# tomer196/GaUDI

Measured on AMD Instinct MI355X. Metric: guided molecules/sec (1000-step), higher is better.
Workload: dtype f32

## Files before the change

### gaudi_amd/csrc/w8_edm.h

```cpp
#pragma once
#include "edm_device.h"
#include "w8_common.h"
#include "w8_split.h"
#include "w8_nodes_f16.h"

namespace gaudi {
namespace w8 {

__host__ __device__ constexpr int gn_lds_buffers(int gn) { return gn == 2 ? 2 : 0; }
template <int HP, int SP = 0, int GN = 0>
struct NetSmem {
  static constexpr bool kGlobalNodes = GN != 0;
  float *h, *p, *q;
  float *agg, *agg1;
  float* ring;
  float *x, *x0;
  uint32_t *pmax, *qmax;
  float* hsc;
  f4* geo;
  float* d0;
  float* trans;
  float* vec;
  float* hk = nullptr;
  __host__ __device__ static int floats(int N, int S) {
// ... 126 lines not shown
  __syncthreads();
  compute_geo(sm, mg, 0.f, tid, true);
  typename EdgeRing<HP, SP>::type ring;
  er_init<HP>(ring, sm.ring, W.ktail != 0, W.ws, W.hinv);
  static_assert(SP == 0 || NodeMath<SP>::kF16, "the split edge GEMMs take their column scales from the fp16 node GEMMs' row maxima");
  constexpr bool NH = NodeMath<SP>::kF16;
  constexpr bool RI = node_ring_idle(HP, SP, GN);
  constexpr bool STG = GN && !NH;
  float* const xs0 = sm.ring;
  float* const xs1 = sm.ring + stage_stride(N * LD);
  if constexpr (!RI) er_start<HP>(ring, wbe, lay.gcl(0, 0) + 2 * PK, wave, lane);
  typename NodePFSel<HP, NH>::type pf;
  node_prefetch_x<HP, NH, kAheadOne>(pf, wb, wbe, lay.gcl(0, 0), mg.NC, wave, lane, tw);
  auto hctx = [&]() {
    if constexpr (NH) {
      if constexpr (RI) return node_ctx_h<HP>(sm.ring, EdgeRing<HP, SP>::kFloats, mg.NC, W.hinv, tw, sm.hsc);
      else return node_ctx_h<HP>(ring.slot(ring.par ^ 1), EdgeRing<HP, SP>::kFloats / 2, mg.NC, W.hinv, tw, sm.hsc);
    } else {
      return NodeCtxH{1.f, nullptr, nullptr, tw, nullptr};
    }
  };
  const bool keep = NH && sm.hk != nullptr;
  bool h_kept = false;
  constexpr int NV = (7 * HP + 16 + kThreads - 1) / kThreads;
  VecPF<NV> vpf;
  vec_prefetch<NV, kThreads>(vpf, wb, lay.gcl(0, 0) + 6 * PK, 7 * HP + 16, tid);
  STAMP(ST_EDM_IO);

  for (int l = 0; l < W.L; ++l) {
    compute_geo(sm, mg, W.norm_constant, tid, false);
    STAMP(ST_GEO);
    for (int s = 0; s < W.S; ++s) {
      const int G = lay.gcl(l, s);
      const int Wnext_edge = s + 1 < W.S ? lay.gcl(l, s + 1) + 2 * PK : lay.equ(l) + 2 * PK;
      if constexpr (STG) stage_rows(xs0, sm.h, N * LD, wave, lane);
      for (int idx = tid; idx < N * (LD / 4); idx += kThreads) {
        *(f4*)(sm.agg + 4 * idx) = splat(0.f);
        *(f4*)(sm.agg1 + 4 * idx) = splat(0.f);
      }
      if (tid < N) {
        sm.pmax[tid] = 0u;
        sm.qmax[tid] = 0u;
      }
      vec_commit<NV, kThreads>(vpf, sm.vec, 7 * HP + 16, tid);
      if constexpr (STG) stage_wait();
      else __syncthreads();
      STAMP(ST_STAGE);
      const float *cr = sm.vec, *cd = sm.vec + HP, *b1 = sm.vec + 2 * HP, *b2 = sm.vec + 3 * HP, *wa = sm.vec + 4 * HP,
                  *bn1 = sm.vec + 5 * HP, *bn2 = sm.vec + 6 * HP;
      const float ba = sm.vec[7 * HP];
      const float crmax = sm.vec[7 * HP + 1], cdmax = sm.vec[7 * HP + 2];
      {
        const NodeCtxH cx = keep ? node_ctx_keep<HP>(hctx(), sm.hk, mg.NC) : hctx();
        node_gemm_x<HP, EPI_NONE, false, GN, NH, kAheadOne, kAheadAll, FL>(wb, wbe, G, sm.h, xs0, !h_kept, -1, nullptr, nullptr, b1, sm.p, nullptr, nullptr, mg.NC,
                                                      wave, lane, tw, cx, pf, G + PK, nullptr, sm.pmax);
        h_kept = keep;
        node_gemm_x<HP, EPI_NONE, false, GN, NH, kAheadAll, kAheadOne, FL>(wb, wbe, G + PK, sm.h, xs0, false, -1, nullptr, nullptr, nullptr, sm.q, nullptr,
                                                      nullptr, mg.NC, wave, lane, tw, cx, pf,
                                                      G + 3 * PK, nullptr, sm.qmax);
      }
      STAMP(ST_NODE);
      __syncthreads();
      STAMP(ST_BARRIER);
      if constexpr (RI) er_start<HP>(ring, wbe, G + 2 * PK, wave, lane);
      for (int rd = 0; rd < mg.rounds; ++rd) {
        const TileCols tc = load_tile(mg, rd, wave, c);
        const f4 gg = sm.geo[tc.slot];
        f4 acc[T];
        const float d0v = sm.d0[tc.slot];
        const float ub = __builtin_bit_cast(float, sm.pmax[tc.i]) + __builtin_bit_cast(float, sm.qmax[tc.j]) + crmax * gg[0] + cdmax * fabsf(d0v);
        er_gemm_pq<HP>(acc, ring, wbe, G + 2 * PK, rd + 1 < mg.rounds ? G + 2 * PK : (RI ? -1 : Wnext_edge), b2, cr, cd,
                         sm.p + tc.i * LD + 4 * g, sm.q + tc.j * LD + 4 * g, gg[0], d0v, ub, tc.active, wave, lane STAMP_ARGS);
        STAMP(ST_EDGE);
        if (tc.active) {
          float sdot = 0.f;
#pragma unroll
          for (int t = 0; t < T; ++t) {
            const f4 m = silu4v(acc[t]);
            acc[t] = m;
            const f4 wv = *(const f4*)(wa + 16 * t + 4 * g);
            sdot += m[0] * wv[0] + m[1] * wv[1] + m[2] * wv[2] + m[3] * wv[3];
          }
          float a = 1.f;
          if (W.attention) a = sigmoid_f(reduce_groups(sdot) + ba);
          const float sc = a * tc.mk;
#pragma unroll
          for (int t = 0; t < T; ++t) acc[t] = acc[t] * sc;
          scatter_runs<HP>(acc, tc, sm.agg, sm.agg1, g);
        }
        STAMP(ST_EDGE_EPI);
      }
      __syncthreads();
      STAMP(ST_BARRIER);
      constexpr bool SUM = NH && GN == 0;
      if constexpr (!SUM) {
        if constexpr (STG) stage_rows(xs0, sm.h, N * LD, wave, lane);
        for (int idx = tid; idx < N * (HP / 4); idx += kThreads) {
          const int n = idx / (HP / 4), f = 4 * (idx % (HP / 4));
          if constexpr (STG)
            *(f4*)(xs1 + n * LD + f) = (*(const f4*)(sm.agg + n * LD + f) + *(const f4*)(sm.agg1 + n * LD + f)) / W.normf;
          else
            *(f4*)(sm.agg + n * LD + f) = (*(const f4*)(sm.agg + n * LD + f) + *(const f4*)(sm.agg1 + n * LD + f)) / W.normf;
        }
        if constexpr (STG) stage_wait();
        else __syncthreads();
      }
      STAMP(ST_MISC);
      node_gemm_x<HP, EPI_SILU, true, GN, NH, kAheadOne, kAheadOne, FL, SUM ? 2 : 0>(
          wb, wbe, G + 3 * PK, sm.h, xs0, !h_kept, G + 4 * PK, sm.agg, xs1, bn1, sm.p, nullptr, nullptr, mg.NC, wave, lane, tw,
          keep ? node_ctx_keep<HP>(hctx(), sm.hk, mg.NC) : hctx(), pf, G + 5 * PK, nullptr, nullptr, sm.agg1, W.normf);
      STAMP(ST_NODE);
      __syncthreads();
      STAMP(ST_BARRIER);
      vec_prefetch<NV, kThreads>(vpf, wb, s + 1 < W.S ? lay.gcl(l, s + 1) + 6 * PK : lay.equ(l) + 3 * PK,
                                 s + 1 < W.S ? 7 * HP + 16 : 5 * HP + 16, tid);
      if constexpr (STG) {
        stage_rows(xs0, sm.p, N * LD, wave, lane);
        stage_wait();
      }
      node_gemm_x<HP, EPI_RESIDUAL_MASK, false, GN, NH, kAheadOne, kAheadOne, FL>(wb, wbe, G + 5 * PK, sm.p, xs0, true, -1, nullptr, nullptr, bn2, sm.h, sm.h, mg.mask,
                                                       mg.NC, wave, lane, tw, hctx(), pf,
                                                       s + 1 < W.S ? lay.gcl(l, s + 1) : lay.equ(l));
      h_kept = false;
      STAMP(ST_NODE);
      __syncthreads();
      STAMP(ST_BARRIER);
    }
    {
      const int E = lay.equ(l);
      const int Wnext_edge = l + 1 < W.L ? lay.gcl(l + 1, 0) + 2 * PK : -1;
      vec_commit<NV, kThreads>(vpf, sm.vec, 5 * HP + 16, tid);
      if (tid < N) {
        sm.pmax[tid] = 0u;
        sm.qmax[tid] = 0u;
      }
      if constexpr (STG) {
        stage_rows(xs0, sm.h, N * LD, wave, lane);
        stage_wait();
      } else {
        __syncthreads();
      }
      STAMP(ST_STAGE);
      const float *cr = sm.vec, *cd = sm.vec + HP, *b1 = sm.vec + 2 * HP, *b2 = sm.vec + 3 * HP, *w3 = sm.vec + 4 * HP;
      const float crmax = sm.vec[5 * HP], cdmax = sm.vec[5 * HP + 1];
      {
        const NodeCtxH cx = keep ? node_ctx_keep<HP>(hctx(), sm.hk, mg.NC) : hctx();
        node_gemm_x<HP, EPI_NONE, false, GN, NH, kAheadOne, kAheadAll, FL>(wb, wbe, E, sm.h, xs0, !h_kept, -1, nullptr, nullptr, b1, sm.p, nullptr, nullptr, mg.NC,
                                                      wave, lane, tw, cx, pf, E + PK, nullptr, sm.pmax);
        h_kept = keep;
// ... 96 lines not shown
```

### gaudi_amd/csrc/w8_nodes_f16.h

```cpp
#pragma once
#include "w8_split.h"

namespace gaudi {
namespace w8 {


constexpr float kLoScale = 2048.f;
#ifndef GAUDI_NODE_ABLATE
#define GAUDI_NODE_ABLATE 0
#endif
constexpr int kAblateH = GAUDI_NODE_ABLATE;
#ifndef GAUDI_NODE_STAMPS
#define GAUDI_NODE_STAMPS 0
#endif
#ifndef GAUDI_NODE_PRIO
#define GAUDI_NODE_PRIO 1
#endif
struct NodeStampH {
  unsigned long long sum[8], last;
  __device__ __forceinline__ void start() { last = __builtin_amdgcn_s_memtime(); }
  __device__ __forceinline__ void mark(int i) {
    const unsigned long long t = __builtin_amdgcn_s_memtime();
    sum[i] += t - last;
    last = t;
// ... 55 lines not shown
};
template <bool DIV>
struct RowsSum {
  const float *a, *b;
  float d;
  __device__ __forceinline__ f4 load(int off) const {
    const f4 s = *(const f4*)(a + off) + *(const f4*)(b + off);
    return DIV ? s / d : s;
  }
};
__device__ __forceinline__ RowsOne rows_of(const float* x) { return RowsOne{x}; }
__device__ __forceinline__ RowsOne rows_of(const RowsOne& r) { return r; }
__device__ __forceinline__ RowsOne rows_of(decltype(nullptr)) { return RowsOne{nullptr}; }
template <bool DIV>
__device__ __forceinline__ RowsSum<DIV> rows_of(const RowsSum<DIV>& r) { return r; }
template <int HP, class SRC>
__device__ __forceinline__ SplitRowH split_row_load(const SRC& X, int n, int lane) {
  constexpr int LD = HP + 4;
  SplitRowH r;
  r.x = lane < HP / 4 ? X.load(n * LD + 4 * lane) : splat(0.f);
  r.mx = umax(umax(absbits(r.x[0]), absbits(r.x[1])), umax(absbits(r.x[2]), absbits(r.x[3])));
  return r;
}
template <int HP>
__device__ __forceinline__ void split_row_store(const SplitBufH& sb, const f4 x, uint32_t mx, int n, int lane) {
  constexpr int T = HP / 16, nc = nh_chunks(HP);
  const int m = lane >> 3, g = (lane >> 1) & 3, half = lane & 1;
  int k = 141 - (int)(mx >> 23);
  k = k > 126 ? 126 : k;
  const float s = __builtin_bit_cast(float, (uint32_t)(k + 127) << 23), inv = __builtin_bit_cast(float, (uint32_t)(127 - k) << 23);
  const float y0 = x[0] * s, y1 = x[1] * s, y2 = x[2] * s, y3 = x[3] * s;
  const uint32_t h01 = pk_f16(y0, y1), h23 = pk_f16(y2, y3);
  const f2 f01 = unpk_f16(h01), f23 = unpk_f16(h23);
  const uint32_t l01 = pk_f16((y0 - f01[0]) * kLoScale, (y1 - f01[1]) * kLoScale),
                 l23 = pk_f16((y2 - f23[0]) * kLoScale, (y3 - f23[1]) * kLoScale);
  const int ct = n >> 4, c = n & 15;
  if (m < nc) {
    float* d = sb.chunk(m) + ct * 512 + nh_bpos(c, g) + half * 2;
    *(u2*)d = (u2){h01, h23};
    *(u2*)(d + 256) = (u2){l01, l23};
  } else if (nh_odd(HP) && lane < HP / 4) {
    float* d = sb.tail(HP) + ct * 256 + 4 * (lane - 4 * (T - 1)) * 16 + c;
    d[0] = x[0];
    d[16] = x[1];
    d[32] = x[2];
    d[48] = x[3];
  }
  if (lane == 0) sb.scale(HP)[ct * 16 + c] = inv;
}
template <int HP, class SRC>
__device__ __forceinline__ void split_rows_h(const SplitBufH& sb, const SRC& X_, int N, int wave, int lane) {
  const auto X = rows_of(X_);
  for (int n = wave; n < N; n += 2 * kWaves) {
    const int n2 = n + kWaves < N ? n + kWaves : n;
    SplitRowH a = split_row_load<HP>(X, n, lane), b = split_row_load<HP>(X, n2, lane);
    a.mx = wave_max_u32(a.mx);
    b.mx = wave_max_u32(b.mx);
    split_row_store<HP>(sb, a.x, a.mx, n, lane);
    if (n2 != n) split_row_store<HP>(sb, b.x, b.mx, n2, lane);
  }
}

__device__ __forceinline__ void lds_barrier() {
  asm volatile("s_waitcnt lgkmcnt(0)" ::: "memory");
  __builtin_amdgcn_s_barrier();
  asm volatile("" ::: "memory");
}

#ifndef GAUDI_NODE_DEPTH
#define GAUDI_NODE_DEPTH 3
#endif
#ifndef GAUDI_NODE_LATE
#define GAUDI_NODE_LATE 0
#endif
#ifndef GAUDI_NODE_TAIL_EARLY
#define GAUDI_NODE_TAIL_EARLY 0
#endif
template <int HP>
struct NodeGeoH {
  static constexpr int T = HP / 16;
  static constexpr int NTW = T > kWaves ? 2 : 1;
  static constexpr int nc = nh_chunks(HP);
  static constexpr int D = nc < GAUDI_NODE_DEPTH ? (nc > 0 ? nc : 1) : GAUDI_NODE_DEPTH;
  static constexpr bool odd = nh_odd(HP);
};
template <int NTW>
struct NodeSetH {
  u4 p[NTW][2];
};
template <int HP>
struct NodePFH {
// ... 22 lines not shown
template <int HP, int AHEAD = kAheadAll>
__device__ __forceinline__ void node_prefetch_h(NodePFH<HP>& pf, const WBuf& wh, int W , int wave, int lane) {
  constexpr int nd = AHEAD < NodeGeoH<HP>::D ? AHEAD : NodeGeoH<HP>::D;
  const TileLanesH<HP> tl(wave, lane);
  static_for<nd>([&](auto d_tag) {
    constexpr int d = decltype(d_tag)::value;
    nh_load<HP>(pf.s[d], wh, 2 * W + d * nh_chunk_floats(HP), tl);
  });
}

constexpr int kNodePlain = 0;
constexpr int kNodeFresh = 1;
constexpr int kNodeOneTile = 2;
constexpr int kTailRuntime = 0;
constexpr int kTailOne = 1;

struct NodeCtxH {
  float winv;
  float* split_a;
  float* split_b;
  bool ktail;
  float* scales;
  float* scales_b = nullptr;
};

struct YInitBias {};
struct YInitRows {
  const float* y;
};
template <int HP, int EPI, bool TWO, int MAXNT, int PIN = kAheadOne, int POUT = kAheadOne, int FL = kNodePlain, int TAIL = kTailRuntime,
          int NU = 0, class XB = const float*, class XA = const float*, class YI = YInitBias>
__device__ __forceinline__ void node_gemm_h(const WBuf& wh, int Wa, const XA& sXa, bool do_split_a, int Wb, const XB& sXb,
                                            const float* sBias, float* sY, const float* sRes, const float* sMask, int N, int wave,
                                            int lane, const NodeCtxH& cx, NodePFH<HP>& pf, int nextW = -1, float* gPre = nullptr,
                                            uint32_t* sMaxOut = nullptr ,
                                            NodeStampH* ns = nullptr, const YI& yinit = YI{}) {
  (void)ns;
  (void)yinit;
  using G = NodeGeoH<HP>;
  constexpr int T = G::T, LD = HP + 4, NTW = NU > 0 ? NU : G::NTW, nc = G::nc, D = G::D;
  constexpr int kIn = PIN < D ? PIN : D, kOut = POUT < D ? POUT : D;
  constexpr int kLate = nc < D ? 0 : (GAUDI_NODE_LATE < kOut ? GAUDI_NODE_LATE : kOut);
  constexpr int TQ = TAIL == kTailOne ? 1 : 4;
  const bool ktail = TAIL == kTailOne ? true : cx.ktail;
  constexpr bool kFresh = FL == kNodeFresh;
  const int c = lane & 15, g = lane >> 4;
  const int nt = (MAXNT < 2 || N <= 16) ? 1 : (MAXNT < 3 || N <= 32) ? 2 : 3;
  const bool seq = TWO && cx.split_b == cx.split_a;
  const SplitBufH sa{cx.split_a, nt, cx.scales}, sb{cx.split_b, nt, cx.scales_b != nullptr ? cx.scales_b : cx.scales + kScaleFloatsH};
  const int bpos = nh_bpos(c, g);
  const TileLanesH<HP> tl(wave, lane);
  const TileLanesH<HP> tl_next(wave, lane, nextW >= 0);
  const int Wn = nextW >= 0 ? nextW : Wa;
  static_for<D>([&](auto d_tag) {
    constexpr int d = decltype(d_tag)::value;
    if constexpr (d >= kIn) nh_load<HP, NTW>(pf.s[d], wh, 2 * Wa + d * nh_chunk_floats(HP), tl);
  });
  float ta[NTW][TQ], tb[NTW][TQ];
  if constexpr (G::odd) {
#pragma unroll
    for (int u = 0; u < NTW; ++u) {
      const int t = wave + kWaves * u < T ? wave + kWaves * u : 0;
#pragma unroll
      for (int q = 0; q < TQ; ++q) {
        const int ln = ((q == 0 || !ktail) && wave + kWaves * u < T) ? lane : kOOBLane;
        ta[u][q] = __builtin_bit_cast(float, __builtin_amdgcn_raw_buffer_load_b32(wh.r, ln * 4, (2 * Wa + nh_tail_off(HP) + t * 256 + q * 64) * 4, 0));
        if constexpr (TWO)
          tb[u][q] = __builtin_bit_cast(float, __builtin_amdgcn_raw_buffer_load_b32(wh.r, ln * 4, (2 * Wb + nh_tail_off(HP) + t * 256 + q * 64) * 4, 0));
      }
    }
  }
  NSTAMP(0);
  if (!(kAblateH & 1)) {
    const int ls = kFresh ? fresh(lane) : lane;
    if (do_split_a) split_rows_h<HP>(sa, rows_of(sXa), N, wave, ls);
    if (TWO && !seq) split_rows_h<HP>(sb, sXb, N, wave, ls);
    NSTAMP(1);
    if (do_split_a || (TWO && !seq)) lds_barrier();
    NSTAMP(2);
  }

  f4 acc0[MAXNT][NTW], acc1[MAXNT][NTW], y[MAXNT][NTW];
#pragma unroll
  for (int j = 0; j < MAXNT; ++j)
#pragma unroll
    for (int u = 0; u < NTW; ++u) {
      const int t = wave + kWaves * u < T ? wave + kWaves * u : 0;
      acc0[j][u] = splat(0.f);
      acc1[j][u] = splat(0.f);
      y[j][u] = sBias != nullptr ? *(const f4*)(sBias + 16 * t + 4 * g) : splat(0.f);
      if constexpr (std::is_same<YI, YInitRows>::value)
        y[j][u] = j * 16 + c < N ? *(const f4*)(yinit.y + (j * 16 + c) * LD + 16 * t + 4 * g) : splat(0.f);
    }
  struct BH {
    u4 h, l;
  };
  auto bld = [&](const SplitBufH& s_, int i, int j) {
    const float* q = s_.chunk(i) + bpos + j * 512;
    return BH{*(const u4*)q, *(const u4*)(q + 256)};
  };
  auto mm = [&](const NodeSetH<G::NTW>& s, const BH& b, int j) {
// ... 93 lines not shown
  source(std::integral_constant<int, 0>{}, sa);
  NSTAMP(4);
  if constexpr (!TWO) late(std::integral_constant<int, kOut - kLate>{});
  fold(sa, ta);
  NSTAMP(5);
  if constexpr (TWO) {
    if (seq) {
      lds_barrier();
      split_rows_h<HP>(sb, sXb, N, wave, kFresh ? fresh(lane) : lane);
      lds_barrier();
    }
    tail_early(sb, tb);
    source(std::integral_constant<int, 1>{}, sb);
    late(std::integral_constant<int, kOut - kLate>{});
    fold(sb, tb);
  }
  static_for<D>([&](auto d_tag) {
    if constexpr (decltype(d_tag)::value > kOut - kLate) late(d_tag);
  });
#if GAUDI_NODE_PRIO
  if constexpr (!kFresh) __builtin_amdgcn_s_setprio(0);
#endif
  const int le = kFresh ? fresh(lane) : lane, ce = le & 15, ge = le >> 4;
  static_for<MAXNT>([&](auto j_tag) {
    constexpr int j = decltype(j_tag)::value;
    if (j < nt) {
#pragma unroll
      for (int u = 0; u < NTW; ++u) {
        const int t = wave + kWaves * u;
        const int nd = j * 16 + ce;
        f4 yy = y[j][u];
        if (t < T && nd < N) {
          float* dst = sY + nd * LD + 16 * t + 4 * ge;
          const bool pad = G::odd && ktail && t == T - 1 && ge > 0;
          if (pad) yy = splat(0.f);
          if (gPre != nullptr) nstash_store((f4*)(gPre + nd * HP + 16 * t + 4 * ge), yy);
          if (sMaxOut != nullptr) atomicMax(sMaxOut + nd, umax(umax(absbits(yy[0]), absbits(yy[1])), umax(absbits(yy[2]), absbits(yy[3]))));
          if (!pad) {
            if (EPI == EPI_SILU) yy = silu4v(yy);
            if (EPI == EPI_RESIDUAL_MASK) {
              const f4 r = *(const f4*)(sRes + nd * LD + 16 * t + 4 * ge);
              yy = (r + yy) * sMask[nd];
            }
            if (EPI == EPI_MUL_DSILU) {
              const f4 r = *(const f4*)(sRes + nd * LD + 16 * t + 4 * ge);
              yy = yy * dsilu4v(r);
            }
            if (EPI == EPI_ACCUM) yy = *(const f4*)(sRes + nd * LD + 16 * t + 4 * ge) + yy;
          }
          *(f4*)dst = yy;
        }
      }
    }
  });
  NSTAMP(6);
}

template <int HP>
struct SideGeoH {
  static constexpr int T = HP / 16, nc = nh_chunks(HP), TG = 7;
  static constexpr int NG = (T + TG - 1) / TG;
  static constexpr int kSteps = NG * nc;
  static constexpr bool odd = nh_odd(HP);
  static_assert(nc >= 1, "at least one fp16 chunk");
  __host__ __device__ static constexpr int tiles(int gq) { return (gq + 1) * TG <= T ? TG : T - gq * TG; }
  __host__ __device__ static constexpr int loads(int s) {
    return (s < 0 || s >= kSteps) ? 0 : tiles(s / nc) * (2 + ((odd && s % nc == nc - 1) ? 1 : 0));
  }
};
template <int HP>
struct SideJobH {
  using G = SideGeoH<HP>;
  u4 w[G::TG][2];
// ... 82 lines not shown
  });
}

#ifndef GAUDI_NODE_F16
#define GAUDI_NODE_F16 1
#endif
template <int SP>
struct NodeMath {
  static constexpr bool kF16 = SP != 0 && GAUDI_NODE_F16 != 0;
};
template <int HP, bool NH>
struct NodePFSel {
  using type = NodePF<HP>;
};
template <int HP>
struct NodePFSel<HP, true> {
  using type = NodePFH<HP>;
};
template <int HP, bool NH, int AHEAD, class PF>
__device__ __forceinline__ void node_prefetch_x(PF& pf, const WBuf& wb, const WBuf& wbe, int W, int N, int wave, int lane, bool tw) {
  if constexpr (NH) node_prefetch_h<HP, AHEAD>(pf, wbe, W, wave, lane);
  else node_prefetch<HP>(pf, wb, W, wave, lane, tw);
}
template <int HP, int EPI, bool TWO, int GN, bool NH, int PIN, int POUT, int FL = kNodePlain, int XBS = 0, class PF>
__device__ __forceinline__ void node_gemm_x(const WBuf& wb, const WBuf& wbe, int Wa, const float* Xa, const float* XaS, bool split_a, int Wb,
                                            const float* Xb, const float* XbS, const float* sBias, float* sY, const float* sRes,
                                            const float* sMask, int N, int wave, int lane, bool tw, const NodeCtxH& cx, PF& pf,
                                            int nextW = -1, float* gPre = nullptr, uint32_t* sMaxOut = nullptr,
                                            const float* Xb1 = nullptr, float xb_div = 1.f) {
  static_assert(XBS == 0 || (NH && GN == 0 && TWO), "summed second sources: the fp16-pair form of the resident kernels");
  if constexpr (NH) {
    constexpr int MAXNT = GN ? 3 : FL == kNodeOneTile ? 1 : 2;
    constexpr int TAIL = FL == kNodeOneTile && nh_odd(HP) ? kTailOne : kTailRuntime;
    if constexpr (XBS == 0)
      node_gemm_h<HP, EPI, TWO, MAXNT, PIN, POUT, FL, TAIL>(wbe, Wa, Xa, split_a, Wb, Xb, sBias, sY, sRes, sMask, N, wave, lane, cx, pf, nextW,
                                                            gPre, sMaxOut);
    else
      node_gemm_h<HP, EPI, TWO, MAXNT, PIN, POUT, FL, TAIL>(wbe, Wa, Xa, split_a, Wb, RowsSum<XBS == 2>{Xb, Xb1, xb_div}, sBias, sY, sRes, sMask, N,
                                                            wave, lane, cx, pf, nextW, gPre, sMaxOut);
  } else if constexpr (GN != 0) {
    node_gemm_n<HP, EPI, true, 3>(wb, Wa, XaS, Wb, XbS, sBias, sY, sRes, sMask, N, wave, lane, tw, &pf, nextW, gPre);
  } else {
    node_gemm<HP, EPI, true>(wb, Wa, Xa, Wb, Xb, sBias, sY, sRes, sMask, N, wave, lane, tw, &pf, nextW, gPre);
  }
}
__host__ __device__ constexpr bool node_ring_idle(int HP, int SP, bool GN) {
  return GN || (SP != 0 && GAUDI_NODE_F16 != 0 && (SP == 2 || HP < 48));
}
template <int HP>
__device__ __forceinline__ NodeCtxH node_ctx_h(float* region, int cap, int N, float winv, bool ktail, float* scales) {
  const int nct = N <= 16 ? 1 : N <= 32 ? 2 : 3;
  const int need = nh_split_floats(HP, nct);
  return NodeCtxH{winv, region, 2 * need <= cap ? region + need : region, ktail, scales};
}
__host__ __device__ constexpr int nh_keep_floats(int HP, int N) { return nh_split_floats(HP, N <= 16 ? 1 : N <= 32 ? 2 : 3) + kScaleFloatsH; }
template <int HP>
__device__ __forceinline__ NodeCtxH node_ctx_keep(const NodeCtxH& cx, float* keep, int N) {
  const int nct = N <= 16 ? 1 : N <= 32 ? 2 : 3;
  return NodeCtxH{cx.winv, keep + kScaleFloatsH, cx.split_a, cx.ktail, keep, cx.scales};
  (void)nct;
}

// ... 3 lines not shown
```

### gaudi_amd/csrc/w8_pred.h

```cpp
#pragma once
#include "pred_device.h"
#include "w8_edm.h"

namespace gaudi {
namespace w8 {

template <int HP, int SP = 0, int GN = 0, bool PG = false>
struct PredSmem {
  static_assert(!(PG && GN != 0), "PG is a variant of the resident kernels");
  static_assert(!GN || SP != 0, "global node buffers: split edge GEMMs only (the fp32 form's publish buffer starts in b0 / b1)");
  static constexpr bool kGlobalNodes = GN != 0;
  float *b2, *b3, *b4;
  float *b0, *b1;
  float* ring;
  float* pub;
  float *x, *x0, *dx;
  uint32_t *pmax, *qmax;
  float* hsc;
  f4* geo;
  float *d0, *trans, *dd0;
  float* pred;
  float* vec;
  float* hk = nullptr;
  float* side = nullptr;
// ... 76 lines not shown
    }
  }
  __syncthreads();
  compute_geo(sm, mg, 0.f, tid, true);
  typename EdgeRing<HP, SP>::type ring;
  er_init<HP>(ring, sm.ring, W.ktail != 0, W.ws, W.hinv);
  constexpr bool NH = NodeMath<SP>::kF16;
  constexpr bool RI = node_ring_idle(HP, SP, GN);
  constexpr bool STG = GN && !NH;
  float* const xs0 = sm.ring;
  float* const xs1 = sm.ring + stage_stride(N * LD);
  if constexpr (!RI) er_start<HP>(ring, wbe, lay.layer(0) + 2 * HP * HP, wave, lane);
  typename NodePFSel<HP, NH>::type pf;
  node_prefetch_x<HP, NH, kAheadOne>(pf, wb, wbe, lay.layer(0), mg.NC, wave, lane, tw);
  auto hctx = [&]() {
    if constexpr (NH) {
      if constexpr (RI) return node_ctx_h<HP>(sm.ring, EdgeRing<HP, SP>::kFloats, mg.NC, W.hinv, tw, sm.hsc);
      else return node_ctx_h<HP>(ring.slot(ring.par ^ 1), EdgeRing<HP, SP>::kFloats / 2, mg.NC, W.hinv, tw, sm.hsc);
    } else {
      return NodeCtxH{1.f, nullptr, nullptr, tw, nullptr};
    }
  };
  const bool keep = NH && sm.hk != nullptr;
  constexpr bool kSideA = (SD & 1) != 0;
  static_assert(!kSideA || (NH && !MR && GN == 0 && !RI && FL == kNodeOneTile), "the side job is a form of the resident N1 kernel");
  constexpr int NV = (PredLayerW::vec_count(HP) + kThreads - 1) / kThreads;
  VecPF<NV> vpf;
  vec_prefetch<NV, kThreads>(vpf, wb, PredLayerW::vec_off(lay.layer(0), HP), PredLayerW::vec_count(HP), tid);

  for (int l = 0; l < W.L; ++l) {
    const bool last = l == W.L - 1;
    const PredLayerW Lw(w, lay.layer(l), HP, sm.vec);
    const bool side_l = kSideA && sm.side != nullptr && !last && (tw || !SplitGeo<HP, SP == 0 ? 1 : SP>::kTailOK);
    vec_commit<NV, kThreads>(vpf, sm.vec, PredLayerW::vec_count(HP), tid);
    if constexpr (STG) stage_rows(xs0, h, N * LD, wave, lane);
    for (int idx = tid; idx < N * LD; idx += kThreads) {
      agg[idx] = 0.f;
      agg1[idx] = 0.f;
    }
    if (tid < N) {
      sm.pmax[tid] = 0u;
      sm.qmax[tid] = 0u;
    }
    float* st = stash + (size_t)l * (3 * N * HP + 4 * N);
    for (int idx = tid; idx < N; idx += kThreads) gstore4((f4*)(st + 3 * N * HP) + idx, *(const f4*)(sm.x + 4 * idx));
    compute_geo(sm, mg, 1.0f, tid, false);
    if constexpr (STG) stage_wait();
    else __syncthreads();
    STAMP(ST_STAGE);
    {
      const NodeCtxH cx = keep ? node_ctx_keep<HP>(hctx(), sm.hk, mg.NC) : hctx();
      node_gemm_x<HP, EPI_NONE, false, GN, NH, kAheadOne, kAheadAll, FL>(wb, wbe, Lw.A, h, xs0, true, -1, nullptr, nullptr, Lw.b1, p, nullptr, nullptr, mg.NC, wave,
                                                    lane, tw, cx, pf, Lw.Bm, nullptr, sm.pmax);
      node_gemm_x<HP, EPI_NONE, false, GN, NH, kAheadAll, kAheadOne, FL>(wb, wbe, Lw.Bm, h, xs0, false, -1, nullptr, nullptr, nullptr, q, nullptr, nullptr, mg.NC,
                                                    wave, lane, tw, cx, pf, side_l ? Lw.Wn1a : Lw.Wn1h, nullptr, sm.qmax);
    }
    STAMP(ST_NODE);
    __syncthreads();
    STAMP(ST_BARRIER);
    if constexpr (RI) er_start<HP>(ring, wbe, Lw.W2, wave, lane);
    for (int idx = tid; idx < N * (HP / 4); idx += kThreads) {
      const int n = idx / (HP / 4), f = 4 * (idx % (HP / 4));
      nstash_store((f4*)st + idx, *(const f4*)(p + n * LD + f));
      nstash_store((f4*)(st + N * HP) + idx, *(const f4*)(q + n * LD + f));
    }
    STAMP(ST_STASH);
    int rd = 0;
    if (side_l && wave == kWaves - 1) {
      if constexpr (kSideA) {
        constexpr int n = side_trip_count<HP, SP>();
        SideJobH<HP> job;
        const SideArgsH sa{wbe, Lw.Wn1h, Lw.bn1, SplitBufH{sm.hk + kScaleFloatsH, 1, sm.hk}, W.hinv, sm.side, mg.NC};
        side_issue<HP, 0>(job, sa, lane);
        side_trips<HP, SP, 0>(ring, wbe, split_off(Lw.W2), split_off(Lw.Wc1), lane, job, sa);
        side_trips<HP, SP, n>(ring, wbe, split_off(Lw.Wc1), split_off(lay.layer(l + 1) + 2 * HP * HP), lane, job, sa);
        side_rest<HP, 2 * n>(job, sa, lane);
      }
    } else
    {
    pred_fwd_round:
      const bool more = MR && rd + 1 < mg.rounds;
      const TileCols tc = load_tile(mg, MR ? rd : 0, wave, c);
      const f4 gg = sm.geo[tc.slot];
// ... 53 lines not shown
        if (++rd < mg.rounds) goto pred_fwd_round;
      }
    }
    __syncthreads();
    STAMP(ST_BARRIER);
    constexpr bool SUM = NH && GN == 0;
    if constexpr (!SUM) {
      if constexpr (STG) stage_rows(xs0, h, N * LD, wave, lane);
      for (int idx = tid; idx < N * (HP / 4); idx += kThreads) {
        const int n = idx / (HP / 4), f = 4 * (idx % (HP / 4));
        if constexpr (STG)
          *(f4*)(xs1 + n * LD + f) = *(const f4*)(agg + n * LD + f) + *(const f4*)(agg1 + n * LD + f);
        else
          *(f4*)(agg + n * LD + f) = *(const f4*)(agg + n * LD + f) + *(const f4*)(agg1 + n * LD + f);
      }
      if constexpr (STG) stage_wait();
      else __syncthreads();
    }
    STAMP(ST_MISC);
    if constexpr (kSideA) {
      if (side_l)
        node_gemm_h<HP, EPI_SILU, false, 1, kAheadOne, kAheadOne, FL, nh_odd(HP) ? kTailOne : kTailRuntime>(
            wbe, Lw.Wn1a, RowsSum<false>{agg, agg1, 1.f}, true, -1, (const float*)nullptr, nullptr, p, nullptr, nullptr, mg.NC, wave, lane,
            hctx(), pf, Lw.Wn2, st + 2 * N * HP , nullptr, nullptr, YInitRows{sm.side});
    }
    if (!side_l)
    node_gemm_x<HP, EPI_SILU, true, GN, NH, kAheadOne, kAheadOne, FL, SUM ? 1 : 0>(
        wb, wbe, Lw.Wn1h, h, xs0, !keep, Lw.Wn1a, agg, xs1, Lw.bn1, p, nullptr, nullptr, mg.NC, wave, lane, tw,
        keep ? node_ctx_keep<HP>(hctx(), sm.hk, mg.NC) : hctx(), pf, Lw.Wn2, st + 2 * N * HP , nullptr, agg1);
    STAMP(ST_NODE);
    __syncthreads();
    STAMP(ST_BARRIER);
    vec_prefetch<NV, kThreads>(vpf, wb, PredLayerW::vec_off(lay.layer(l + 1 < W.L ? l + 1 : l), HP), PredLayerW::vec_count(HP), tid);
    if constexpr (STG) {
      stage_rows(xs0, p, N * LD, wave, lane);
      stage_wait();
    }
    node_gemm_x<HP, EPI_RESIDUAL_MASK, false, GN, NH, kAheadOne, kAheadOne, FL>(wb, wbe, Lw.Wn2, p, xs0, true, -1, nullptr, nullptr, Lw.bn2, h, h, mg.mask, mg.NC, wave,
                                                     lane, tw, hctx(), pf, l + 1 < W.L ? lay.layer(l + 1) : -1);
    if (!last) coord_update(sm, mg, 1.0f, tid);
    STAMP(ST_NODE);
    __syncthreads();
    STAMP(ST_BARRIER);
  }
  {
    const float* ow = w + lay.out_w();
    const float* ob = w + lay.out_b();
    const float* msk = mg.mask;
    small_dots<kThreads>(
        N * K, HP, tid, [=](int qq, int f) { return gload(ow + (qq % K) * HP + f); },
        [=](int qq, int f) { return h[(qq / K) * LD + f]; },
        [=](int qq, float acc) { p[qq] = (acc + gload(ob + qq % K)) * msk[qq / K]; });
    __syncthreads();
    if (tid < K) {
      float s = 0.f;
      for (int n = 0; n < N; ++n) s += p[n * K + tid];
      sm.pred[tid] = s / readout_div;
    }
    __syncthreads();
  }
  STAMP(ST_X0);
}
// ... 46 lines not shown
  __syncthreads();

  typename EdgeRing<HP, SP>::type ring;
  er_init<HP>(ring, sm.ring, W.ktail != 0, W.ws, W.hinv);
  constexpr bool NH = NodeMath<SP>::kF16;
  constexpr bool RI = node_ring_idle(HP, SP, GN);
  constexpr bool STG = GN && !NH;
  float* const xs0 = sm.ring;
  float* const xs1 = sm.ring + stage_stride(N * LD);
  if constexpr (!RI) {
    const int L0 = lay.layer(W.L - 1);
    er_start<HP>(ring, wbe, L0 + 9 * HP * HP , wave, lane);
  }
  typename NodePFSel<HP, NH>::type pf;
  node_prefetch_x<HP, NH, kAheadOne>(pf, wb, wbe, lay.layer(W.L - 1) + 13 * HP * HP , mg.NC, wave, lane, tw);
  auto hctx = [&]() {
    if constexpr (NH) {
      if constexpr (RI) return node_ctx_h<HP>(sm.ring, EdgeRing<HP, SP>::kFloats, mg.NC, W.hinv, tw, sm.hsc);
      else return node_ctx_h<HP>(ring.slot(ring.par ^ 1), EdgeRing<HP, SP>::kFloats / 2, mg.NC, W.hinv, tw, sm.hsc);
    } else {
      return NodeCtxH{1.f, nullptr, nullptr, tw, nullptr};
    }
  };
  constexpr int NV = (PredLayerW::vec_count(HP) + kThreads - 1) / kThreads;
  VecPF<NV> vpf;
  vec_prefetch<NV, kThreads>(vpf, wb, PredLayerW::vec_off(lay.layer(W.L - 1), HP), PredLayerW::vec_count(HP), tid);
  STAMP(ST_X1);
  for (int l = W.L - 1; l >= 0; --l) {
    const bool last = l == W.L - 1;
    const PredLayerW Lw(w, lay.layer(l), HP, sm.vec);
    const float* st = stash + (size_t)l * (3 * N * HP + 4 * N);
    {
      const int tid = fresh(tid_);
      const int n4 = N * (HP / 4);
#ifdef GAUDI_DIAG_HOT_STASH
      const f4* sp = (const f4*)W.w;
      const f4* sq = (const f4*)(W.w + N * HP);
      const f4* sn = (const f4*)(W.w + 2 * N * HP);
#else
      const f4* sp = (const f4*)st;
      const f4* sq = (const f4*)(st + N * HP);
      const f4* sn = (const f4*)(st + 2 * N * HP);
#endif
      const int i0 = tid < n4 ? tid : n4 - 1, i1 = tid + kThreads < n4 ? tid + kThreads : n4 - 1;
      const f4 xv = gload4((const f4*)(st + 3 * N * HP) + (tid < N ? tid : N - 1));
      const f4 p0 = nstash_load(sp + i0), q0 = nstash_load(sq + i0), v0 = nstash_load(sn + i0);
      const f4 p1 = nstash_load(sp + i1), q1 = nstash_load(sq + i1), v1 = nstash_load(sn + i1);
      vec_commit<NV, kThreads>(vpf, sm.vec, PredLayerW::vec_count(HP), tid);
      STAMP(ST_GUIDE);
      auto put = [&](int idx, f4 pv, f4 qv, f4 nv) {
        const int n = idx / (HP / 4), f = 4 * (idx % (HP / 4));
        *(f4*)(B2 + n * LD + f) = pv;
        *(f4*)(B1 + n * LD + f) = qv;
        *(f4*)(B4 + n * LD + f) = nv;
        *(f4*)(dh + n * LD + f) = *(const f4*)(dh + n * LD + f) * mg.mask[n];
      };
      if (tid < N) {
        *(f4*)(sm.x + 4 * tid) = xv;
        *(f4*)(sm.dx + 4 * tid) = *(const f4*)(sm.dx + 4 * tid) * mg.mask[tid];
      }
      if (tid < n4) put(tid, p0, q0, v0);
      if (tid + kThreads < n4) put(tid + kThreads, p1, q1, v1);
      for (int idx = tid + 2 * kThreads; idx < n4; idx += kThreads) put(idx, nstash_load(sp + idx), nstash_load(sq + idx), nstash_load(sn + idx));
      for (int idx = tid + kThreads; idx < N; idx += kThreads) {
        *(f4*)(sm.x + 4 * idx) = gload4((const f4*)(st + 3 * N * HP) + idx);
        *(f4*)(sm.dx + 4 * idx) = *(const f4*)(sm.dx + 4 * idx) * mg.mask[idx];
      }
    }
    STAMP(ST_PRED_IO);
    __syncthreads();
    if constexpr (STG) stage_rows(xs0, dh, N * LD, wave, lane);
    compute_geo(sm, mg, 1.0f, tid, false);
    if constexpr (STG) stage_wait();
    STAMP(ST_BWD_EDGE);
    node_gemm_x<HP, EPI_MUL_DSILU, false, GN, NH, kAheadOne, kAheadOne, FL>(wb, wbe, Lw.Wn2t, dh, xs0, true, -1, nullptr, nullptr, nullptr, STG ? xs1 : B4, B4, nullptr,
                                                 mg.NC, wave, lane, tw, hctx(), pf, Lw.Wn1ht);
    __syncthreads();
    {
      const NodeCtxH cx = hctx();
      node_gemm_x<HP, EPI_ACCUM, false, GN, NH, kAheadOne, kAheadAll, FL>(wb, wbe, Lw.Wn1ht, B4, xs1, true, -1, nullptr, nullptr, nullptr, dh, dh, nullptr, mg.NC,
                                                     wave, lane, tw, cx, pf, Lw.Wn1at);
      node_gemm_x<HP, EPI_NONE, false, GN, NH, kAheadAll, 0, FL>(wb, wbe, Lw.Wn1at, B4, xs1, false, -1, nullptr, nullptr, nullptr, B0, nullptr, nullptr,
                                                    mg.NC, wave, lane, tw, cx, pf);
    }
    __syncthreads();
    STAMP(ST_BWD_NODE);
    if constexpr (RI) er_start<HP>(ring, wbe, last ? Lw.W2t : Lw.Wc1t, wave, lane);
    {
      constexpr bool mr = MR;
      int rd = 0;
    pred_bwd_round:
      const bool more = MR && rd + 1 < mg.rounds;
      const TileCols tc = load_tile(mg, MR ? rd : 0, wave, c);
      const int tile = tc.slot >> 4;
      const f4 gg = sm.geo[tc.slot];
      const float d0v = sm.d0[tc.slot];
      f4 du[T];
      float a = 0.f, tau = 0.f, dtx = 0.f, dty = 0.f, dtz = 0.f;
      {
        f4 de[T];
        if (tc.active) {
          a = gload(astash + (size_t)l * S + tc.slot);
          dtx = sm.dx[4 * tc.i + 0];
          dty = sm.dx[4 * tc.i + 1];
// ... 286 lines not shown
```

Baseline: 224.6.

## Chain node GEMM epilogues directly into fp16 split operand for next GEMM

Adds a chained-epilogue path in which a node GEMM keeps its output rows in registers, reduces per-row absolute maxima with LDS atomics, and after a barrier writes the fp16 hi/lo split operand for the next GEMM directly. The next GEMM then skips its own read-and-split pass over the activations. This is applied to the EDM node MLP (p and h chains), to the predictor forward, and to the predictor backward dsilu→accum chain, enabled by default through GAUDI_CHAIN=7 for one-tile resident kernels. It costs extra registers for the held rows, atomics and an extra LDS barrier, and the chained path must reproduce the original split layout exactly.

```diff
diff --git a/gaudi_amd/csrc/w8_edm.h b/gaudi_amd/csrc/w8_edm.h
--- a/gaudi_amd/csrc/w8_edm.h
+++ b/gaudi_amd/csrc/w8_edm.h
@@ -172,6 +172,11 @@
   };
   const bool keep = NH && sm.hk != nullptr;
   bool h_kept = false;
+  constexpr bool kChainP = NH && FL == kNodeOneTile && (GAUDI_CHAIN & 1) != 0, kChainH = NH && FL == kNodeOneTile && (GAUDI_CHAIN & 2) != 0;
+  constexpr bool kChain = kChainP || kChainH;
+  [[maybe_unused]] uint32_t* const mxp = (uint32_t*)sm.hsc + 16;
+  [[maybe_unused]] uint32_t* const mxh = (uint32_t*)sm.hsc + 32;
+  [[maybe_unused]] ChainRowsH<HP> crow;
   constexpr int NV = (7 * HP + 16 + kThreads - 1) / kThreads;
   VecPF<NV> vpf;
   vec_prefetch<NV, kThreads>(vpf, wb, lay.gcl(0, 0) + 6 * PK, 7 * HP + 16, tid);
@@ -213,6 +218,12 @@
       __syncthreads();
       STAMP(ST_BARRIER);
       if constexpr (RI) er_start<HP>(ring, wbe, G + 2 * PK, wave, lane);
+      if constexpr (kChain) {
+        if (tid < 16) {
+          mxp[tid] = 0u;
+          mxh[tid] = 0u;
+        }
+      }
       for (int rd = 0; rd < mg.rounds; ++rd) {
         const TileCols tc = load_tile(mg, rd, wave, c);
         const f4 gg = sm.geo[tc.slot];
@@ -256,25 +267,50 @@
         else __syncthreads();
       }
       STAMP(ST_MISC);
+      if constexpr (kChainP)
+        node_gemm_x<HP, EPI_SILU, true, GN, NH, kAheadOne, kAheadOne, FL, SUM ? 2 : 0>(
+            wb, wbe, G + 3 * PK, sm.h, xs0, !h_kept, G + 4 * PK, sm.agg, xs1, bn1, sm.p, nullptr, nullptr, mg.NC, wave, lane, tw,
+            keep ? node_ctx_keep<HP>(hctx(), sm.hk, mg.NC) : hctx(), pf, G + 5 * PK, nullptr, nullptr, sm.agg1, W.normf,
+            ChainOutH<HP, false>{&crow, mxp});
+      else
       node_gemm_x<HP, EPI_SILU, true, GN, NH, kAheadOne, kAheadOne, FL, SUM ? 2 : 0>(
           wb, wbe, G + 3 * PK, sm.h, xs0, !h_kept, G + 4 * PK, sm.agg, xs1, bn1, sm.p, nullptr, nullptr, mg.NC, wave, lane, tw,
           keep ? node_ctx_keep<HP>(hctx(), sm.hk, mg.NC) : hctx(), pf, G + 5 * PK, nullptr, nullptr, sm.agg1, W.normf);
       STAMP(ST_NODE);
       __syncthreads();
       STAMP(ST_BARRIER);
+      if constexpr (kChainP) {
+        const NodeCtxH cx = hctx();
+        chain_split_store<HP>(SplitBufH{cx.split_a, 1, cx.scales}, crow, mxp, mg.NC, wave, lane);
+      }
       vec_prefetch<NV, kThreads>(vpf, wb, s + 1 < W.S ? lay.gcl(l, s + 1) + 6 * PK : lay.equ(l) + 3 * PK,
                                  s + 1 < W.S ? 7 * HP + 16 : 5 * HP + 16, tid);
       if constexpr (STG) {
         stage_rows(xs0, sm.p, N * LD, wave, lane);
         stage_wait();
       }
+      if constexpr (kChain) {
+        NodeCtxH cx = hctx();
+        cx.chained = kChainP;
+        node_gemm_x<HP, EPI_RESIDUAL_MASK, false, GN, NH, kAheadOne, kAheadOne, FL>(wb, wbe, G + 5 * PK, sm.p, xs0, !kChainP, -1, nullptr, nullptr, bn2, sm.h, sm.h,
+                                                         mg.mask, mg.NC, wave, lane, tw, cx, pf,
+                                                         s + 1 < W.S ? lay.gcl(l, s + 1) : lay.equ(l), nullptr, nullptr, nullptr, 1.f,
+                                                         ChainOutH<HP, true>{&crow, kChainH && keep ? mxh : nullptr});
+      } else {
       node_gemm_x<HP, EPI_RESIDUAL_MASK, false, GN, NH, kAheadOne, kAheadOne, FL>(wb, wbe, G + 5 * PK, sm.p, xs0, true, -1, nullptr, nullptr, bn2, sm.h, sm.h, mg.mask,
                                                        mg.NC, wave, lane, tw, hctx(), pf,
                                                        s + 1 < W.S ? lay.gcl(l, s + 1) : lay.equ(l));
+      }
       h_kept = false;
       STAMP(ST_NODE);
       __syncthreads();
       STAMP(ST_BARRIER);
+      if constexpr (kChainH) {
+        if (keep) {
+          chain_split_store<HP>(SplitBufH{sm.hk + kScaleFloatsH, 1, sm.hk}, crow, mxh, mg.NC, wave, lane);
+          h_kept = true;
+        }
+      }
     }
     {
       const int E = lay.equ(l);
diff --git a/gaudi_amd/csrc/w8_nodes_f16.h b/gaudi_amd/csrc/w8_nodes_f16.h
--- a/gaudi_amd/csrc/w8_nodes_f16.h
+++ b/gaudi_amd/csrc/w8_nodes_f16.h
@@ -101,10 +101,11 @@
   r.mx = umax(umax(absbits(r.x[0]), absbits(r.x[1])), umax(absbits(r.x[2]), absbits(r.x[3])));
   return r;
 }
-template <int HP>
-__device__ __forceinline__ void split_row_store(const SplitBufH& sb, const f4 x, uint32_t mx, int n, int lane) {
-  constexpr int T = HP / 16, nc = nh_chunks(HP);
-  const int m = lane >> 3, g = (lane >> 1) & 3, half = lane & 1;
+struct SplitPiecesH {
+  uint32_t h01, h23, l01, l23;
+  float inv;
+};
+__device__ __forceinline__ SplitPiecesH split_pieces(const f4 x, uint32_t mx) {
   int k = 141 - (int)(mx >> 23);
   k = k > 126 ? 126 : k;
   const float s = __builtin_bit_cast(float, (uint32_t)(k + 127) << 23), inv = __builtin_bit_cast(float, (uint32_t)(127 - k) << 23);
@@ -113,11 +114,18 @@
   const f2 f01 = unpk_f16(h01), f23 = unpk_f16(h23);
   const uint32_t l01 = pk_f16((y0 - f01[0]) * kLoScale, (y1 - f01[1]) * kLoScale),
                  l23 = pk_f16((y2 - f23[0]) * kLoScale, (y3 - f23[1]) * kLoScale);
+  return SplitPiecesH{h01, h23, l01, l23, inv};
+}
+template <int HP>
+__device__ __forceinline__ void split_row_store(const SplitBufH& sb, const f4 x, uint32_t mx, int n, int lane) {
+  constexpr int T = HP / 16, nc = nh_chunks(HP);
+  const int m = lane >> 3, g = (lane >> 1) & 3, half = lane & 1;
+  const SplitPiecesH pc = split_pieces(x, mx);
   const int ct = n >> 4, c = n & 15;
   if (m < nc) {
     float* d = sb.chunk(m) + ct * 512 + nh_bpos(c, g) + half * 2;
-    *(u2*)d = (u2){h01, h23};
-    *(u2*)(d + 256) = (u2){l01, l23};
+    *(u2*)d = (u2){pc.h01, pc.h23};
+    *(u2*)(d + 256) = (u2){pc.l01, pc.l23};
   } else if (nh_odd(HP) && lane < HP / 4) {
     float* d = sb.tail(HP) + ct * 256 + 4 * (lane - 4 * (T - 1)) * 16 + c;
     d[0] = x[0];
@@ -125,7 +133,7 @@
     d[32] = x[2];
     d[48] = x[3];
   }
-  if (lane == 0) sb.scale(HP)[ct * 16 + c] = inv;
+  if (lane == 0) sb.scale(HP)[ct * 16 + c] = pc.inv;
 }
 template <int HP, class SRC>
 __device__ __forceinline__ void split_rows_h(const SplitBufH& sb, const SRC& X_, int N, int wave, int lane) {
@@ -146,6 +154,52 @@
   asm volatile("" ::: "memory");
 }
 
+#ifndef GAUDI_CHAIN
+#define GAUDI_CHAIN 7
+#endif
+template <int HP>
+struct ChainRowsH {
+  f4 y[HP / 16 > kWaves ? 2 : 1];
+};
+struct ChainNoneH {
+  static constexpr bool kOn = false, kStore = true;
+};
+template <int HP, bool STORE>
+struct ChainOutH {
+  static constexpr bool kOn = true, kStore = STORE;
+  ChainRowsH<HP>* rows;
+  uint32_t* mx;
+};
+__device__ __forceinline__ bool co_off(const ChainNoneH&) { return true; }
+template <int HP, bool STORE>
+__device__ __forceinline__ bool co_off(const ChainOutH<HP, STORE>& co) { return co.mx == nullptr; }
+template <int HP>
+__device__ __forceinline__ void chain_split_store(const SplitBufH& sb, const ChainRowsH<HP>& r, const uint32_t* mx, int N, int wave, int lane) {
+  constexpr int T = HP / 16, NTW = T > kWaves ? 2 : 1;
+  const int c = lane & 15, g = lane >> 4;
+  if (c >= N) return;
+  const uint32_t m = mx[c];
+#pragma unroll
+  for (int u = 0; u < NTW; ++u) {
+    const int t = wave + kWaves * u;
+    if (t >= T) continue;
+    const f4 x = r.y[u];
+    const SplitPiecesH pc = split_pieces(x, m);
+    if (nh_odd(HP) && t == T - 1) {
+      float* d = sb.tail(HP) + 4 * g * 16 + c;
+      d[0] = x[0];
+      d[16] = x[1];
+      d[32] = x[2];
+      d[48] = x[3];
+    } else {
+      float* d = sb.chunk(t >> 1) + nh_bpos(c, 2 * (t & 1) + (g >> 1)) + (g & 1) * 2;
+      *(u2*)d = (u2){pc.h01, pc.h23};
+      *(u2*)(d + 256) = (u2){pc.l01, pc.l23};
+    }
+    if (t == 0 && g == 0) sb.scale(HP)[c] = pc.inv;
+  }
+}
+
 #ifndef GAUDI_NODE_DEPTH
 #define GAUDI_NODE_DEPTH 3
 #endif
@@ -214,6 +268,7 @@
   bool ktail;
   float* scales;
   float* scales_b = nullptr;
+  bool chained = false;
 };
 
 struct YInitBias {};
@@ -221,14 +276,16 @@
   const float* y;
 };
 template <int HP, int EPI, bool TWO, int MAXNT, int PIN = kAheadOne, int POUT = kAheadOne, int FL = kNodePlain, int TAIL = kTailRuntime,
-          int NU = 0, class XB = const float*, class XA = const float*, class YI = YInitBias>
+          int NU = 0, class XB = const float*, class XA = const float*, class YI = YInitBias, class CO = ChainNoneH>
 __device__ __forceinline__ void node_gemm_h(const WBuf& wh, int Wa, const XA& sXa, bool do_split_a, int Wb, const XB& sXb,
                                             const float* sBias, float* sY, const float* sRes, const float* sMask, int N, int wave,
                                             int lane, const NodeCtxH& cx, NodePFH<HP>& pf, int nextW = -1, float* gPre = nullptr,
                                             uint32_t* sMaxOut = nullptr ,
-                                            NodeStampH* ns = nullptr, const YI& yinit = YI{}) {
+                                            NodeStampH* ns = nullptr, const YI& yinit = YI{}, const CO& co = CO{}) {
   (void)ns;
   (void)yinit;
+  (void)co;
+  static_assert(!CO::kOn || (MAXNT == 1 && FL != kNodeFresh), "chained epilogues: the kernels of one column tile");
   using G = NodeGeoH<HP>;
   constexpr int T = G::T, LD = HP + 4, NTW = NU > 0 ? NU : G::NTW, nc = G::nc, D = G::D;
   constexpr int kIn = PIN < D ? PIN : D, kOut = POUT < D ? POUT : D;
@@ -268,7 +325,7 @@
     if (do_split_a) split_rows_h<HP>(sa, rows_of(sXa), N, wave, ls);
     if (TWO && !seq) split_rows_h<HP>(sb, sXb, N, wave, ls);
     NSTAMP(1);
-    if (do_split_a || (TWO && !seq)) lds_barrier();
+    if (do_split_a || (TWO && !seq) || cx.chained) lds_barrier();
     NSTAMP(2);
   }
 
@@ -408,6 +465,11 @@
   if constexpr (!kFresh) __builtin_amdgcn_s_setprio(0);
 #endif
   const int le = kFresh ? fresh(lane) : lane, ce = le & 15, ge = le >> 4;
+  if constexpr (CO::kOn) {
+    if (co.mx != nullptr)
+#pragma unroll
+      for (int u = 0; u < NTW; ++u) co.rows->y[u] = splat(0.f);
+  }
   static_for<MAXNT>([&](auto j_tag) {
     constexpr int j = decltype(j_tag)::value;
     if (j < nt) {
@@ -434,7 +496,13 @@
             }
             if (EPI == EPI_ACCUM) yy = *(const f4*)(sRes + nd * LD + 16 * t + 4 * ge) + yy;
           }
-          *(f4*)dst = yy;
+          if constexpr (CO::kOn) {
+            if (co.mx != nullptr) {
+              atomicMax(co.mx + nd, umax(umax(absbits(yy[0]), absbits(yy[1])), umax(absbits(yy[2]), absbits(yy[3]))));
+              co.rows->y[u] = yy;
+            }
+          }
+          if (CO::kStore || co_off(co)) *(f4*)dst = yy;
         }
       }
     }
@@ -563,22 +631,23 @@
   if constexpr (NH) node_prefetch_h<HP, AHEAD>(pf, wbe, W, wave, lane);
   else node_prefetch<HP>(pf, wb, W, wave, lane, tw);
 }
-template <int HP, int EPI, bool TWO, int GN, bool NH, int PIN, int POUT, int FL = kNodePlain, int XBS = 0, class PF>
+template <int HP, int EPI, bool TWO, int GN, bool NH, int PIN, int POUT, int FL = kNodePlain, int XBS = 0, class PF, class CO = ChainNoneH>
 __device__ __forceinline__ void node_gemm_x(const WBuf& wb, const WBuf& wbe, int Wa, const float* Xa, const float* XaS, bool split_a, int Wb,
                                             const float* Xb, const float* XbS, const float* sBias, float* sY, const float* sRes,
                                             const float* sMask, int N, int wave, int lane, bool tw, const NodeCtxH& cx, PF& pf,
                                             int nextW = -1, float* gPre = nullptr, uint32_t* sMaxOut = nullptr,
-                                            const float* Xb1 = nullptr, float xb_div = 1.f) {
+                                            const float* Xb1 = nullptr, float xb_div = 1.f, const CO& co = CO{}) {
+  static_assert(!CO::kOn || NH, "chained epilogues: the fp16-pair form");
   static_assert(XBS == 0 || (NH && GN == 0 && TWO), "summed second sources: the fp16-pair form of the resident kernels");
   if constexpr (NH) {
     constexpr int MAXNT = GN ? 3 : FL == kNodeOneTile ? 1 : 2;
     constexpr int TAIL = FL == kNodeOneTile && nh_odd(HP) ? kTailOne : kTailRuntime;
     if constexpr (XBS == 0)
       node_gemm_h<HP, EPI, TWO, MAXNT, PIN, POUT, FL, TAIL>(wbe, Wa, Xa, split_a, Wb, Xb, sBias, sY, sRes, sMask, N, wave, lane, cx, pf, nextW,
-                                                            gPre, sMaxOut);
+                                                            gPre, sMaxOut, nullptr, YInitBias{}, co);
     else
       node_gemm_h<HP, EPI, TWO, MAXNT, PIN, POUT, FL, TAIL>(wbe, Wa, Xa, split_a, Wb, RowsSum<XBS == 2>{Xb, Xb1, xb_div}, sBias, sY, sRes, sMask, N,
-                                                            wave, lane, cx, pf, nextW, gPre, sMaxOut);
+                                                            wave, lane, cx, pf, nextW, gPre, sMaxOut, nullptr, YInitBias{}, co);
   } else if constexpr (GN != 0) {
     node_gemm_n<HP, EPI, true, 3>(wb, Wa, XaS, Wb, XbS, sBias, sY, sRes, sMask, N, wave, lane, tw, &pf, nextW, gPre);
   } else {
diff --git a/gaudi_amd/csrc/w8_pred.h b/gaudi_amd/csrc/w8_pred.h
--- a/gaudi_amd/csrc/w8_pred.h
+++ b/gaudi_amd/csrc/w8_pred.h
@@ -122,6 +122,9 @@
     }
   };
   const bool keep = NH && sm.hk != nullptr;
+  constexpr bool kChainP = NH && FL == kNodeOneTile && (GAUDI_CHAIN & 1) != 0;
+  [[maybe_unused]] uint32_t* const mxp = (uint32_t*)sm.hsc + 16;
+  [[maybe_unused]] ChainRowsH<HP> crow;
   constexpr bool kSideA = (SD & 1) != 0;
   static_assert(!kSideA || (NH && !MR && GN == 0 && !RI && FL == kNodeOneTile), "the side job is a form of the resident N1 kernel");
   constexpr int NV = (PredLayerW::vec_count(HP) + kThreads - 1) / kThreads;
@@ -159,6 +162,9 @@
     __syncthreads();
     STAMP(ST_BARRIER);
     if constexpr (RI) er_start<HP>(ring, wbe, Lw.W2, wave, lane);
+    if constexpr (kChainP) {
+      if (tid < 16) mxp[tid] = 0u;
+    }
     for (int idx = tid; idx < N * (HP / 4); idx += kThreads) {
       const int n = idx / (HP / 4), f = 4 * (idx % (HP / 4));
       nstash_store((f4*)st + idx, *(const f4*)(p + n * LD + f));
@@ -258,22 +264,41 @@
       if (side_l)
         node_gemm_h<HP, EPI_SILU, false, 1, kAheadOne, kAheadOne, FL, nh_odd(HP) ? kTailOne : kTailRuntime>(
             wbe, Lw.Wn1a, RowsSum<false>{agg, agg1, 1.f}, true, -1, (const float*)nullptr, nullptr, p, nullptr, nullptr, mg.NC, wave, lane,
-            hctx(), pf, Lw.Wn2, st + 2 * N * HP , nullptr, nullptr, YInitRows{sm.side});
-    }
+            hctx(), pf, Lw.Wn2, st + 2 * N * HP , nullptr, nullptr, YInitRows{sm.side}, ChainOutH<HP, !kChainP>{&crow, kChainP ? mxp : nullptr});
+    }
+    if constexpr (kChainP) {
+      if (!side_l)
+        node_gemm_x<HP, EPI_SILU, true, GN, NH, kAheadOne, kAheadOne, FL, SUM ? 1 : 0>(
+            wb, wbe, Lw.Wn1h, h, xs0, !keep, Lw.Wn1a, agg, xs1, Lw.bn1, p, nullptr, nullptr, mg.NC, wave, lane, tw,
+            keep ? node_ctx_keep<HP>(hctx(), sm.hk, mg.NC) : hctx(), pf, Lw.Wn2, st + 2 * N * HP , nullptr, agg1, 1.f,
+            ChainOutH<HP, false>{&crow, mxp});
+    } else {
     if (!side_l)
     node_gemm_x<HP, EPI_SILU, true, GN, NH, kAheadOne, kAheadOne, FL, SUM ? 1 : 0>(
         wb, wbe, Lw.Wn1h, h, xs0, !keep, Lw.Wn1a, agg, xs1, Lw.bn1, p, nullptr, nullptr, mg.NC, wave, lane, tw,
         keep ? node_ctx_keep<HP>(hctx(), sm.hk, mg.NC) : hctx(), pf, Lw.Wn2, st + 2 * N * HP , nullptr, agg1);
+    }
     STAMP(ST_NODE);
     __syncthreads();
     STAMP(ST_BARRIER);
+    if constexpr (kChainP) {
+      const NodeCtxH cx = hctx();
+      chain_split_store<HP>(SplitBufH{cx.split_a, 1, cx.scales}, crow, mxp, mg.NC, wave, lane);
+    }
     vec_prefetch<NV, kThreads>(vpf, wb, PredLayerW::vec_off(lay.layer(l + 1 < W.L ? l + 1 : l), HP), PredLayerW::vec_count(HP), tid);
     if constexpr (STG) {
       stage_rows(xs0, p, N * LD, wave, lane);
       stage_wait();
     }
+    if constexpr (kChainP) {
+      NodeCtxH cx = hctx();
+      cx.chained = true;
+      node_gemm_x<HP, EPI_RESIDUAL_MASK, false, GN, NH, kAheadOne, kAheadOne, FL>(wb, wbe, Lw.Wn2, p, xs0, false, -1, nullptr, nullptr, Lw.bn2, h, h, mg.mask, mg.NC,
+                                                       wave, lane, tw, cx, pf, l + 1 < W.L ? lay.layer(l + 1) : -1);
+    } else {
     node_gemm_x<HP, EPI_RESIDUAL_MASK, false, GN, NH, kAheadOne, kAheadOne, FL>(wb, wbe, Lw.Wn2, p, xs0, true, -1, nullptr, nullptr, Lw.bn2, h, h, mg.mask, mg.NC, wave,
                                                      lane, tw, hctx(), pf, l + 1 < W.L ? lay.layer(l + 1) : -1);
+    }
     if (!last) coord_update(sm, mg, 1.0f, tid);
     STAMP(ST_NODE);
     __syncthreads();
@@ -366,6 +391,8 @@
       return NodeCtxH{1.f, nullptr, nullptr, tw, nullptr};
     }
   };
+  constexpr bool kChain = NH && FL == kNodeOneTile && (GAUDI_CHAIN & 4) != 0;
+  [[maybe_unused]] uint32_t* const mxd = (uint32_t*)sm.hsc + 16;
   constexpr int NV = (PredLayerW::vec_count(HP) + kThreads - 1) / kThreads;
   VecPF<NV> vpf;
   vec_prefetch<NV, kThreads>(vpf, wb, PredLayerW::vec_off(lay.layer(W.L - 1), HP), PredLayerW::vec_count(HP), tid);
@@ -403,6 +430,9 @@
         *(f4*)(sm.x + 4 * tid) = xv;
         *(f4*)(sm.dx + 4 * tid) = *(const f4*)(sm.dx + 4 * tid) * mg.mask[tid];
       }
+      if constexpr (kChain) {
+        if (tid < 16) mxd[tid] = 0u;
+      }
       if (tid < n4) put(tid, p0, q0, v0);
       if (tid + kThreads < n4) put(tid + kThreads, p1, q1, v1);
       for (int idx = tid + 2 * kThreads; idx < n4; idx += kThreads) put(idx, nstash_load(sp + idx), nstash_load(sq + idx), nstash_load(sn + idx));
@@ -417,13 +447,25 @@
     compute_geo(sm, mg, 1.0f, tid, false);
     if constexpr (STG) stage_wait();
     STAMP(ST_BWD_EDGE);
+    if constexpr (kChain) {
+      ChainRowsH<HP> crow;
+      node_gemm_x<HP, EPI_MUL_DSILU, false, GN, NH, kAheadOne, kAheadOne, FL>(wb, wbe, Lw.Wn2t, dh, xs0, true, -1, nullptr, nullptr, nullptr, B4, B4, nullptr,
+                                                   mg.NC, wave, lane, tw, hctx(), pf, Lw.Wn1ht, nullptr, nullptr, nullptr, 1.f,
+                                                   ChainOutH<HP, false>{&crow, mxd});
+      __syncthreads();
+      const NodeCtxH cx = hctx();
+      chain_split_store<HP>(SplitBufH{cx.split_a, 1, cx.scales}, crow, mxd, mg.NC, wave, lane);
+    } else {
     node_gemm_x<HP, EPI_MUL_DSILU, false, GN, NH, kAheadOne, kAheadOne, FL>(wb, wbe, Lw.Wn2t, dh, xs0, true, -1, nullptr, nullptr, nullptr, STG ? xs1 : B4, B4, nullptr,
                                                  mg.NC, wave, lane, tw, hctx(), pf, Lw.Wn1ht);
     __syncthreads();
+    }
     {
       const NodeCtxH cx = hctx();
-      node_gemm_x<HP, EPI_ACCUM, false, GN, NH, kAheadOne, kAheadAll, FL>(wb, wbe, Lw.Wn1ht, B4, xs1, true, -1, nullptr, nullptr, nullptr, dh, dh, nullptr, mg.NC,
-                                                     wave, lane, tw, cx, pf, Lw.Wn1at);
+      NodeCtxH cx1 = cx;
+      cx1.chained = kChain;
+      node_gemm_x<HP, EPI_ACCUM, false, GN, NH, kAheadOne, kAheadAll, FL>(wb, wbe, Lw.Wn1ht, B4, xs1, !kChain, -1, nullptr, nullptr, nullptr, dh, dh, nullptr, mg.NC,
+                                                     wave, lane, tw, cx1, pf, Lw.Wn1at);
       node_gemm_x<HP, EPI_NONE, false, GN, NH, kAheadAll, 0, FL>(wb, wbe, Lw.Wn1at, B4, xs1, false, -1, nullptr, nullptr, nullptr, B0, nullptr, nullptr,
                                                     mg.NC, wave, lane, tw, cx, pf);
     }
```

New measurement: 225.6, median of 6. About the same (+0.5%).
